# iden3/circom-witnesscalc

Measured on AMD Instinct MI355X. Metric: witnesses/sec, higher is better.
Workload: dtype u32

## Files before the change

### circom-witnesscalc_amd/__init__.py

```python
import ctypes
import os
import subprocess

import numpy as np

_HERE = os.path.dirname(os.path.abspath(__file__))
LIB_PATH = os.environ.get("CWC_LIB_PATH") or os.path.join(_HERE, "libcircom_witnesscalc_amd.so")
_lib = None


class GwStatus(ctypes.Structure):
    _fields_ = [("code", ctypes.c_int), ("error_msg", ctypes.c_void_p)]


class GraphInfo(ctypes.Structure):
    _fields_ = [(n, ctypes.c_uint64) for n in ("n_nodes", "n_op", "n_input_nodes", "n_const", "n_inputs",
                                                "n_witness", "depth", "algorithmic_bytes_per_set")]


class Timing(ctypes.Structure):
    _fields_ = [("tile_width", ctypes.c_uint32), ("n_launches", ctypes.c_uint32), ("n_bundles", ctypes.c_uint64),
                ("n_slots", ctypes.c_uint64), ("interp_ms", ctypes.c_float), ("pack_ms", ctypes.c_float),
                ("divider", ctypes.c_uint32), ("streams", ctypes.c_uint32)]

# ... 17 lines not shown
class Handoff(ctypes.Structure):
    _fields_ = [("struct_size", ctypes.c_uint32), ("form", ctypes.c_uint32), ("hip_stream", ctypes.c_void_p), ("done_event", ctypes.c_void_p)]


FORM_CANONICAL, FORM_MONTGOMERY = 0, 1


class WitnessCalcError(RuntimeError):
    pass


def pinned_rows(shape):
    import weakref
    n = int(np.prod(shape))
    ptr = lib().gwb_host_alloc(n)
    if not ptr:
        raise WitnessCalcError("gwb_host_alloc(%d) failed" % n)
    buf = (ctypes.c_uint8 * max(n, 1)).from_address(ptr)
    weakref.finalize(buf, lib().gwb_host_free, ptr)
    return np.frombuffer(buf, dtype=np.uint8, count=n).reshape(shape)


EXPORTED_SYMBOLS = [
    "gw_calc_witness", "gwb_graph_load", "gwb_graph_free", "gwb_graph_info", "gwb_graph_serialize",
    "gwb_inputs_from_json", "gwb_set_tile_width", "gwb_calc_witness_batch_device", "gwb_calc_witness_batch_host",
    "gwb_last_timing", "gwb_wtns_size", "gwb_wtns_from_witness", "gwb_graph_export", "gwb_graph_import",
    "gwb_free_status", "gwb_profile_classes", "gwb_pick_tile_width", "gwb_inputs_from_json_batch", "gwb_wtns_save_batch",
    "gwb_host_alloc", "gwb_host_free", "gwb_timing_history", "gwb_calc_witness_batch_handoff", "gwb_ubench_modmul", "gwb_graph_pick_tile_width", "gwb_graph_broadcast",
    "gwb_builder_new", "gwb_builder_free", "gwb_builder_input", "gwb_builder_constant", "gwb_builder_uno", "gwb_builder_duo", "gwb_builder_tres",
    "gwb_builder_witness", "gwb_builder_input_signal", "gwb_builder_node_count", "gwb_builder_finish",
    "gwb_ubench_modmul_block", "gwb_program_stats", "gwb_calc_witness_json_to_wtns", "gwb_model_class_cycles",
    "gwb_graphgen_bigint_class", "gwb_graphgen_rsa_long_div_class", "gwb_graph_op_histogram",
    "gwb_kernel_source_hash", "gwb_pack_schedule", "gwb_pack_schedule_of_blob", "gwb_rccl_unique_id", "gwb_rccl_comm_init", "gwb_rccl_comm_ranks", "gwb_rccl_comm_destroy",
]


def build(verbose=False, diag=False):
    cmd = ["make", "-C", os.path.join(_HERE, "csrc"), "-j4"] + (["all", "diag"] if diag else [])
    if not verbose:
        cmd.insert(1, "-s")
    subprocess.check_call(cmd)
    subprocess.check_call(["make"] + ([] if verbose else ["-s"]) + ["-C", os.path.join(_HERE, "r1cs"), "-j4"])


DIAG_LIB_PATH = os.path.join(_HERE, "libcircom_witnesscalc_amd_diag.so")


def lib():
    global _lib
    if _lib is None:
        if not os.path.exists(LIB_PATH):
            raise WitnessCalcError("HIP extension %s is missing: run __graft_entry__.build() "
                                   "(there is no CPU fallback)" % LIB_PATH)
        try:
            import torch
        except ImportError:
            pass
        L = ctypes.CDLL(LIB_PATH)
        vp, sz, u32p = ctypes.c_void_p, ctypes.c_size_t, ctypes.POINTER(ctypes.c_uint32)
        stp = ctypes.POINTER(GwStatus)
        L.gw_calc_witness.restype = ctypes.c_int
        L.gw_calc_witness.argtypes = [ctypes.c_char_p, vp, sz, ctypes.POINTER(vp), ctypes.POINTER(sz), stp]
        L.gwb_graph_load.restype = ctypes.c_int
        L.gwb_graph_load.argtypes = [vp, sz, ctypes.POINTER(vp), stp]
        L.gwb_graph_free.argtypes = [vp]
        L.gwb_graph_info.argtypes = [vp, ctypes.POINTER(GraphInfo)]
        L.gwb_graph_serialize.argtypes = [vp, ctypes.POINTER(vp), ctypes.POINTER(sz), stp]
        L.gwb_inputs_from_json.argtypes = [vp, ctypes.c_char_p, vp, stp]
        L.gwb_set_tile_width.argtypes = [vp, ctypes.c_uint32]
        L.gwb_calc_witness_batch_device.argtypes = [vp, vp, sz, vp, vp, vp, stp]
        L.gwb_calc_witness_batch_host.argtypes = [vp, vp, sz, vp, vp, stp]
        L.gwb_last_timing.argtypes = [vp, ctypes.POINTER(Timing)]
        L.gwb_host_alloc.restype = ctypes.c_void_p
        L.gwb_host_alloc.argtypes = [sz]
        L.gwb_host_free.restype = None
        L.gwb_host_free.argtypes = [ctypes.c_void_p]
        L.gwb_timing_history.restype = ctypes.c_int
        L.gwb_timing_history.argtypes = [ctypes.c_void_p, sz, ctypes.c_void_p, ctypes.c_void_p, ctypes.POINTER(sz)]
        L.gwb_wtns_size.restype = sz
        L.gwb_wtns_size.argtypes = [sz]
        L.gwb_wtns_from_witness.argtypes = [vp, sz, vp]
        L.gwb_graph_export.argtypes = [vp, ctypes.c_uint32, ctypes.POINTER(vp), ctypes.POINTER(sz), stp]
        L.gwb_graph_import.argtypes = [vp, sz, ctypes.POINTER(vp), stp]
        L.gwb_free_status.argtypes = [stp]
        if hasattr(L, "gwb_graphgen_bigint_class"):
            L.gwb_graphgen_bigint_class.argtypes = [ctypes.c_uint32, ctypes.c_uint32, ctypes.c_uint32, ctypes.POINTER(vp), ctypes.POINTER(sz), stp]
            L.gwb_graphgen_rsa_long_div_class.argtypes = [ctypes.c_uint32, ctypes.c_uint32, ctypes.c_uint32, ctypes.c_int, ctypes.POINTER(vp), ctypes.POINTER(sz), stp]
            L.gwb_graph_op_histogram.argtypes = [vp, ctypes.POINTER(ctypes.c_uint64), sz]
        L.gwb_profile_classes.argtypes = [vp, vp, sz, vp, vp, vp, stp]
        L.gwb_inputs_from_json_batch.argtypes = [vp, ctypes.c_char_p, sz, vp, sz, ctypes.POINTER(sz), stp]
        L.gwb_wtns_save_batch.argtypes = [vp, sz, sz, ctypes.c_char_p, stp]
        L.gwb_calc_witness_batch_handoff.argtypes = [vp, vp, sz, vp, vp, ctypes.POINTER(Handoff), stp]
        L.gwb_ubench_modmul.restype = ctypes.c_double
        L.gwb_ubench_modmul.argtypes = [ctypes.c_uint32, ctypes.c_uint32]
        L.gwb_ubench_modmul_block.restype = ctypes.c_double
        L.gwb_model_class_cycles.restype = ctypes.c_double
        L.gwb_kernel_source_hash.restype = ctypes.c_char_p
        L.gwb_kernel_source_hash.argtypes = []
        L.gwb_model_class_cycles.argtypes = [ctypes.c_uint32]
        L.gwb_ubench_modmul_block.argtypes = [ctypes.c_uint32, ctypes.c_uint32]
        L.gwb_program_stats.argtypes = [vp, ctypes.c_uint32, ctypes.POINTER(ProgramStats)]
        if hasattr(L, "gwb_pack_schedule"):
            L.gwb_pack_schedule.argtypes = [vp, ctypes.c_uint32, vp, sz, vp, sz, u32p, u32p, u32p, stp]
            L.gwb_pack_schedule_of_blob.argtypes = [vp, sz, vp, sz, vp, sz, u32p, u32p, u32p, stp]
        L.gwb_calc_witness_json_to_wtns.argtypes = [vp, ctypes.c_char_p, sz, ctypes.c_char_p, sz, ctypes.POINTER(sz), vp, sz, ctypes.POINTER(E2eStats), stp]
        L.gwb_graph_pick_tile_width.restype = ctypes.c_uint32
        L.gwb_graph_pick_tile_width.argtypes = [vp, sz]
        L.gwb_pick_tile_width.restype = ctypes.c_uint32
        L.gwb_pick_tile_width.argtypes = [sz]
        u32 = ctypes.c_uint32
        L.gwb_builder_new.restype = vp
        L.gwb_builder_new.argtypes = []
        L.gwb_builder_free.restype = None
        L.gwb_builder_free.argtypes = [vp]
        for name, args in (("input", [u32]), ("constant", [ctypes.c_char_p, sz]), ("uno", [u32, u32]), ("duo", [u32, u32, u32]), ("tres", [u32, u32, u32, u32])):
            f = getattr(L, "gwb_builder_" + name)
            f.restype = u32
            f.argtypes = [vp] + args
        L.gwb_builder_witness.argtypes = [vp, u32]
        L.gwb_builder_input_signal.argtypes = [vp, ctypes.c_char_p, u32, u32]
        L.gwb_builder_node_count.restype = ctypes.c_uint64
        L.gwb_builder_node_count.argtypes = [vp]
# ... 222 lines not shown
                        done_event.cuda_event if done_event is not None else None)
            rc = lib().gwb_calc_witness_batch_handoff(self._h, d_inputs.data_ptr(), b, d_witness.data_ptr(), d_status.data_ptr(),
                                                      ctypes.byref(h), ctypes.byref(st))
        else:
            rc = lib().gwb_calc_witness_batch_device(self._h, d_inputs.data_ptr(), b, d_witness.data_ptr(),
                                                     d_status.data_ptr(), s.cuda_stream, ctypes.byref(st))
        _check(rc, st)

    def timing_history(self, max_launches):
        a = np.zeros(max_launches, dtype=np.float32)
        b = np.zeros(max_launches, dtype=np.float32)
        n = ctypes.c_size_t(0)
        if lib().gwb_timing_history(self._h, max_launches, a.ctypes.data, b.ctypes.data, ctypes.byref(n)) != 0:
            raise WitnessCalcError("gwb_timing_history failed")
        return a[:n.value], b[:n.value]

    def profile_classes(self, d_inputs, d_witness, d_status):
        out = np.zeros(96, dtype=np.uint64)
        st = GwStatus()
        rc = lib().gwb_profile_classes(self._h, d_inputs.data_ptr(), d_inputs.shape[0], d_witness.data_ptr(),
                                       d_status.data_ptr(), out.ctypes.data, ctypes.byref(st))
        _check(rc, st)
        names = ["INPUT", "MUL", "LIN", "DIV", "CMPZ", "CMPS", "BIT", "IDIVMOD", "TERN", "DIVREQ", "DIVGET", "MULQ"]
        res = {n: tuple(int(x) for x in out[4 * i:4 * i + 4]) for i, n in enumerate(names)}
        res["MULF"] = tuple(int(x) for x in out[64:68])
        res["SCAN"] = tuple(int(x) for x in out[68:72])
        res["_scan_kinds"] = {k: tuple(int(x) for x in out[72 + 4 * i:76 + 4 * i]) for i, k in enumerate(("carry", "division", "convolution", "borrow", "comparison"))}
        res["_sections"] = {"MUL": tuple(int(x) for x in out[48:54]), "LIN": tuple(int(x) for x in out[56:62])}
        res["_issue_part"] = {"MUL": int(out[92]), "LIN": int(out[93])}
        res["_pack"] = {"cycles": int(out[94]), "passes": int(out[95])}
        n = int(out[63])
        res["_waves"] = {"n": n, "max_cycles": int(out[54]), "min_cycles": (1 << 40) - int(out[55]) if n else 0,
                         "mean_cycles": int(out[62]) // n if n else 0}
        return res

    def program_stats(self, key=0):
        ps = ProgramStats()
        if lib().gwb_program_stats(self._h, key, ctypes.byref(ps)) != 0:
            raise WitnessCalcError("gwb_program_stats: no such program")
        n = ps.n_classes
        return {"tile_width": ps.tile_width, "divider": ps.divider, "streams": ps.streams, "n_bundles": ps.n_bundles,
                "n_fused_nodes": ps.n_fused_nodes, "n_scan_steps": ps.n_scan_steps, "n_conv_products": ps.n_conv_products, "chain_floor_cycles": ps.chain_floor_cycles, "model_wave_cycles": ps.model_wave_cycles, "lanes_active_mean": ps.lanes_active_mean, "values_per_bundle_mean": ps.values_per_bundle_mean,
                "class_bundles": {CLASS_NAMES[c]: int(ps.class_bundles[c]) for c in range(n) if ps.class_bundles[c]},
                "class_nodes": {CLASS_NAMES[c]: int(ps.class_nodes[c]) for c in range(n) if ps.class_nodes[c]}}

    def pack_schedule(self, key):
        return _pack_schedule(lambda *a: lib().gwb_pack_schedule(self._h, key, *a))

    def last_timing(self):
        t = Timing()
        if lib().gwb_last_timing(self._h, ctypes.byref(t)) != 0:
            raise WitnessCalcError("gwb_last_timing failed")
        return {n: getattr(t, n) for n, _ in Timing._fields_}


def _pack_schedule(call):
    nw, nr, ni, st = ctypes.c_uint32(), ctypes.c_uint32(), ctypes.c_uint32(), GwStatus()
    _check(call(None, 0, None, 0, ctypes.byref(nw), ctypes.byref(nr), ctypes.byref(ni), ctypes.byref(st)), st)
    order, ready = np.zeros(nw.value, dtype=np.uint32), np.zeros(nr.value, dtype=np.uint32)
    _check(call(order.ctypes.data, order.size, ready.ctypes.data, ready.size, ctypes.byref(nw), ctypes.byref(nr), ctypes.byref(ni), ctypes.byref(st)), st)
    return order, ready, int(ni.value)


def pack_schedule_of_blob(blob):
    blob = bytes(blob)
    return _pack_schedule(lambda *a: lib().gwb_pack_schedule_of_blob(blob, len(blob), *a))
# ... 513 lines not shown
```

### circom-witnesscalc_amd/csrc/capi_batch.cc

```cpp
#include "runtime_internal.hpp"

namespace cwcrt {

int load_graph(const void* data, size_t len, gwb_graph** out, std::string& err) {
    std::unique_ptr<gwb_graph> g(new gwb_graph());
    if (!deserialize_witnesscalc_graph((const uint8_t*)data, len, g->graph, err)) return 1;
    g->has_graph = true;
    Program probe;
    if (!probe_graph(g->graph, probe, err)) return 1;
    g->stats = probe.stats;
    g->n_inputs = probe.n_inputs;
    g->n_witness = probe.n_witness;
    g->inputs = g->graph.inputs;
    g->input_index = g->graph.input_index;
    *out = g.release();
    return 0;
}

}

extern "C" {

void gwb_free_status(gw_status_t* status) {
    if (status && status->error_msg) {
// ... 640 lines not shown
            const double cyc = model_class_cycles((int)c) * (double)p->stats.class_bundles[c];
            const double lanes = (double)p->stats.class_nodes[c] * p->T * ((c == C_MULQ || c == C_MULF) ? (double)COOP_LANES : 1.0);
            wsum += cyc;
            lsum += p->stats.class_bundles[c] ? cyc * lanes / (double)p->stats.class_bundles[c] : 0.0;
            vsum += p->stats.class_bundles[c] ? cyc * (double)p->stats.class_nodes[c] * p->T / (double)p->stats.class_bundles[c] : 0.0;
        }
        out->model_wave_cycles = program_wave_cycles(*p);
        out->lanes_active_mean = wsum > 0 ? lsum / wsum : 0.0;
        out->values_per_bundle_mean = wsum > 0 ? vsum / wsum : 0.0;
        out->n_fused_nodes = p->stats.n_fused_nodes;
        out->chain_floor_cycles = (double)p->stats.chain_floor_cycles;
        out->n_scan_steps = p->stats.n_scan_steps;
        out->n_conv_products = p->stats.n_conv_products;
        return 0;
    } catch (...) {
        return 1;
    }
}

int gwb_timing_history(gwb_graph_t* g, size_t max_launches, float* interp_ms, float* pack_ms, size_t* n_out) {
    if (!g || !n_out || (max_launches && (!interp_ms || !pack_ms))) return 1;
    std::lock_guard<std::mutex> lk(g->mu);
    const size_t n = g->pending.size() < max_launches ? g->pending.size() : max_launches;
    for (size_t i = 0; i < n; ++i) {
        auto& c = g->pending[g->pending.size() - n + i];
        if (hipEventSynchronize(c.after_pack) != hipSuccess || hipEventElapsedTime(&interp_ms[i], c.start, c.after_interp) != hipSuccess ||
            hipEventElapsedTime(&pack_ms[i], c.after_interp, c.after_pack) != hipSuccess)
            return 1;
    }
    *n_out = n;
    return 0;
}

int gwb_profile_classes(gwb_graph_t* g, const void* d_inputs, size_t batch, void* d_witness, uint32_t* d_set_status,
                        uint64_t* out36, gw_status_t* status) {
    return guarded(status, [&]() -> int {
    if (!g || !out36) return fail(status, "null argument");
    if (!gwb_kernels_have_diagnostics())
        return fail(status, "class profiling needs the diagnostic library (make -C circom-witnesscalc_amd/csrc diag; load it with CWC_LIB_PATH=<path of "
                            "libcircom_witnesscalc_amd_diag.so>): the product library carries no stamped interpreter instances");
    std::lock_guard<std::mutex> lk(g->mu);
    std::string err = check_device();
    if (!err.empty()) return fail(status, err);
    unsigned long long* d = nullptr;
    if (hipMalloc(&d, 96 * 8) != hipSuccess || hipMemset(d, 0, 96 * 8) != hipSuccess) return fail(status, "hipMalloc failed");
    g->d_prof = d;
    err = run_device(g, d_inputs, batch, d_witness, d_set_status, nullptr);
    g->d_prof = nullptr;
    if (err.empty() && hipDeviceSynchronize() != hipSuccess) err = "hipDeviceSynchronize failed";
    if (err.empty() && hipMemcpy(out36, d, 96 * 8, hipMemcpyDeviceToHost) != hipSuccess) err = "hipMemcpy failed";
    (void)hipFree(d);
    if (!err.empty()) return fail(status, err);
    set_status(status, OK, "");
    return 0;
    });
}

size_t gwb_wtns_size(size_t n_witness) { return wtns_size(n_witness); }

int gwb_wtns_from_witness(const void* row, size_t n_witness, void* out) {
    if ((!row && n_witness) || !out) return 1;
    wtns_from_witness((const uint8_t*)row, n_witness, (uint8_t*)out);
    return 0;
}

}
```

### circom-witnesscalc_amd/csrc/kernels.hip

```cpp
#include <hip/hip_runtime.h>
#include <stdlib.h>

#include "fr_gfx950.hpp"
#include "scan_gfx950.hpp"
#include "program_dev.h"

namespace cwc {

__device__ __forceinline__ Fr fr_from_u4(const uint4& lo, const uint4& hi) {
    return Fr{{lo.x, lo.y, lo.z, lo.w, hi.x, hi.y, hi.z, hi.w}};
}

__device__ __forceinline__ bool wave_any(bool p) { return __ballot(p) != 0ull; }

struct InterpDims {
    uint32_t n_bundles, n_slots, n_inputs, batch, n_const, n_div_requests, trash_off;
    const uint32_t* div_lanes;
    uint32_t n_streams, stream_first[MAX_STREAMS], stream_count[MAX_STREAMS], stream_div_requests[MAX_STREAMS], stream_cref_first[MAX_STREAMS];
    uint4* pack_out;
    const uint2* pack_entries;
    const uint32_t* pack_ready;
    uint32_t n_inline, pack_mont, n_witness;
};
static const uint32_t ST_DIVIDER_TIMEOUT = 0x80000000u;
// ... 22 lines not shown
    asm volatile("s_mov_b32 m0, %0\n\ts_nop 0\n\tbuffer_load_dwordx4 %1, %2, %3 offen lds"
                 :: "s"(lds_addr), "v"(voff), "s"(rsrc), "s"(soff) : "memory");
}
__device__ __forceinline__ i32x4 make_rsrc_words(const void* base, uint32_t bytes) {
    const uint64_t a = (uint64_t)base;
    return i32x4{(int)(uint32_t)a, (int)((uint32_t)(a >> 32) & 0xffffu), (int)bytes, 0x00020000};
}

template <int T, bool PROF, int W, int PACK, int MODE = 0>
__global__ __launch_bounds__((W > 0 ? (W + 1) * PACK : PACK) * 64) void interp_kernel(const uint32_t* __restrict__ hdr, const uint4* __restrict__ recs,
                                                    const uint32_t* __restrict__ crefs, InterpDims p, WsTable wst,
                                                    const uint4* __restrict__ inputs, uint32_t* __restrict__ status,
                                                    unsigned long long* __restrict__ prof) {
    constexpr int G = 64 / T;
    constexpr bool M2 = MODE == 2 || MODE == 3, WIDE = MODE == 3;
    constexpr uint32_t HI = 16u * T;
    constexpr bool DIVIDER = W > 0;
    constexpr uint32_t NW = (W > 0 ? (uint32_t)W : 1u) * (uint32_t)PACK;
    constexpr uint32_t WD = W > 0 ? (uint32_t)W : 1u;
    constexpr uint32_t AREA = lds_area_bytes((uint32_t)W, LDS_BYTES);
    constexpr uint32_t ML = mbox_lanes((uint32_t)W), MB = mbox_bytes((uint32_t)W);
    const uint32_t batch = p.batch;
    const uint32_t lane = threadIdx.x & 63u;
    const uint32_t wave = (uint32_t)__builtin_amdgcn_readfirstlane((int)(threadIdx.x >> 6));
    const uint32_t n_tiles = (batch + T - 1) / T;
    const uint32_t t = lane % T;
    const uint32_t j = (G == 1) ? 0u : lane / T;
    const uint32_t NS = p.n_streams;
    const uint32_t stream = wave < NW ? wave % NS : 0u;
    const uint32_t tile_raw = blockIdx.x * (NW / NS) + (wave < NW ? wave : 0u) / NS;
    const uint32_t tile = tile_raw < n_tiles ? tile_raw : n_tiles - 1;
    const uint32_t set = tile * T + t;
    const uint32_t set_c = set < batch ? set : batch - 1;
    const uint64_t tile_bytes = ws_tile_bytes(p.n_const, p.n_slots, T);
    const uint32_t chunk = tile / wst.tiles_per_chunk, tile_in_chunk = tile % wst.tiles_per_chunk;
    char* tile_base = reinterpret_cast<char*>(wst.base[chunk]) + (uint64_t)tile_in_chunk * tile_bytes;
    const __amdgpu_buffer_rsrc_t rsrc = __builtin_amdgcn_make_buffer_rsrc(tile_base, 0, (int)(uint32_t)tile_bytes, 0x00020000);
    const i32x4 rsrc_rec = make_rsrc_words(recs, (p.n_bundles + REC_AHEAD) * (uint32_t)G * 16u);
    uint32_t* const sync_words = reinterpret_cast<uint32_t*>(tile_base + ws_sync_offset(p.n_const, p.n_slots, T));
    static_assert(NW + PACK <= 16, "sequence words: 64 bytes");
    __shared__ uint4 lds[(NW * AREA + (DIVIDER ? NW * MB + 64u : 0u)) / 16];
    const uint32_t area = wave * AREA;
    const uint32_t lds0 = (uint32_t)(uintptr_t)(lds_char*)(char*)lds + area;
    const uint32_t t16 = 16u * t, lane16 = 16u * lane, j16 = 16u * j;
    char* const ldsb = reinterpret_cast<char*>(lds) + area;
    char* const mbox_all = reinterpret_cast<char*>(lds) + NW * AREA;
    char* const mbox = mbox_all + (wave < NW ? wave : 0u) * MB;
    volatile uint32_t* const seq = reinterpret_cast<volatile uint32_t*>(mbox_all + NW * MB);
    if (DIVIDER || NW > 1) {
        if (DIVIDER && threadIdx.x < NW + (uint32_t)PACK) seq[threadIdx.x] = 0;
        if (NS > 1 && wave < NW && stream == 0 && lane < MAX_STREAMS && tile_raw < n_tiles) {
            __hip_atomic_store(sync_words + lane, 0u, __ATOMIC_RELAXED, __HIP_MEMORY_SCOPE_AGENT);
            __builtin_amdgcn_fence(__ATOMIC_RELEASE, "agent");
        }
        if (wave < NW && stream == 0 && j == 0 && tile_raw < n_tiles && set < batch) status[set] = 0;
        __syncthreads();
    } else {
        if (j == 0 && tile_raw < n_tiles && set < batch) status[set] = 0;
    }
    if (DIVIDER) {
        if (wave >= NW) {
            const uint32_t first_w = (wave - NW) * WD, first_tile = blockIdx.x * (NW / NS) + first_w / NS;
            if (first_tile >= n_tiles) return;
            const uint32_t n_active = NS > 1 ? 1u : n_tiles - first_tile < WD ? n_tiles - first_tile : WD;
            char* const mbox_d = mbox_all + first_w * MB;
            const uint32_t n_requests = NS > 1 ? p.stream_div_requests[first_w % NS] : p.n_div_requests;
// ... 70 lines not shown
                    break;
                }
                __builtin_amdgcn_fence(__ATOMIC_ACQUIRE, "workgroup");
                const uint32_t lanes_k = p.div_lanes[div_lanes_base + k];
                const uint32_t total = n_active * lanes_k;
                for (uint32_t g0 = 0; g0 < total; g0 += 64u) {
                    const uint32_t g = g0 + lane;
                    const bool valid = g < total;
                    const uint32_t w = valid ? g / lanes_k : 0u, i = valid ? g % lanes_k : 0u;
                    char* mb = mbox_d + w * MB + 16u * i;
                    const uint4* qa = reinterpret_cast<const uint4*>(mb);
                    const uint4* qb = reinterpret_cast<const uint4*>(mb + 32u * ML);
                    Fr a = fr_from_u4(qa[0], qa[ML]), b = fr_from_u4(qb[0], qb[ML]);
                    if (!valid) b = fr_zero();
                    const Fr inv = fr_inv(b);
                    const Fr r = u256_select(u256_is_zero(b), fr_zero(), fr_mul(a, inv));
                    if (valid) {
                        uint4* qr = reinterpret_cast<uint4*>(mb);
                        qr[0] = make_uint4(r.v[0], r.v[1], r.v[2], r.v[3]);
                        qr[ML] = make_uint4(r.v[4], r.v[5], r.v[6], r.v[7]);
                    }
                }
                __builtin_amdgcn_fence(__ATOMIC_RELEASE, "workgroup");
                if (lane == 0) seq[wave] = k + 1;
            }
            if constexpr (W == 1) {
                if (inl) {
                    pk_run(p.pack_ready[n_requests] < p.n_inline ? p.pack_ready[n_requests] : p.n_inline, 0xffffffffu);
                    if (PROF && lane == 0 && first_tile % 64u == 0) {
                        atomicAdd(&prof[94], pk_cycles);
                        atomicAdd(&prof[95], pk_passes);
                    }
                }
            }
            return;
        }
    }
    if (tile_raw >= n_tiles) return;
    uint32_t div_seq = 0;
    uint32_t n_posts = 0, n_waits = 0;
    uint32_t cref_row = p.stream_cref_first[stream];

    auto ld = [&](uint32_t off) -> Fr {
        const u32x4 lo = __builtin_amdgcn_raw_buffer_load_b128(rsrc, (int)off, 0, 0);
        const u32x4 hi = __builtin_amdgcn_raw_buffer_load_b128(rsrc, (int)off + (int)HI, 0, 0);
        return Fr{{lo.x, lo.y, lo.z, lo.w, hi.x, hi.y, hi.z, hi.w}};
    };
    auto ld_lds = [&](uint32_t addr) -> Fr {
        const uint4* q = reinterpret_cast<const uint4*>(ldsb + addr);
        const uint4 lo = q[0], hi = q[LDS_HALF_BYTES / 16];
        return fr_from_u4(lo, hi);
    };
    auto ld_rec2 = [&](uint32_t bundle, uint32_t half) -> uint2 {
        return *reinterpret_cast<const uint2*>(ldsb + LDS_REC_OFF + (bundle % REC_AHEAD) * REC_BYTES + lane16 + 8u * half);
    };
    const uint32_t B0 = p.stream_first[stream], NBND = B0 + p.stream_count[stream];
    if (NBND == B0) return;
    auto clampb = [&](uint32_t b) { return b < NBND ? b : NBND - 1; };
    auto stage_rec = [&](uint32_t bundle) {
        dma16(lds0 + LDS_REC_OFF + (bundle % REC_AHEAD) * REC_BYTES, j16, rsrc_rec, bundle * (uint32_t)G * 16u);
    };
    constexpr uint32_t DMA_BIAS = 3u * LDS_HALF_BYTES;
    const i32x4 rsrc_dma = make_rsrc_words(tile_base - DMA_BIAS, (uint32_t)tile_bytes + DMA_BIAS);
    const uint32_t dma_soff0 = DMA_BIAS, dma_soff1 = DMA_BIAS + HI - LDS_HALF_BYTES, dma_soff2 = DMA_BIAS - 2u * LDS_HALF_BYTES,
                   dma_soff3 = DMA_BIAS + HI - 3u * LDS_HALF_BYTES;
    static_assert(LDS_HALF_BYTES == 1024, "instruction offsets below are written out");
// ... 766 lines not shown
                const uint32_t cr = crefs[(size_t)cref_row * G + j];
                ++cref_row;
                const Fr y = ld(cr + t16);
                r = u256_select(u256_is_zero(a_op), y, b_op);
                break;
            }
            case C_SYNC: {
                r = fr_zero();
                if (h & HDR_POST) {
                    asm volatile("s_waitcnt vmcnt(0)" ::: "memory");
                    ++n_posts;
                    if (lane == 0) __hip_atomic_store(sync_words + stream, n_posts, __ATOMIC_RELEASE, __HIP_MEMORY_SCOPE_AGENT);
                }
                if (h & HDR_WAIT) {
                    ++n_waits;
                    if (!post_wait(sync_words, n_waits)) err_bits |= ST_SYNC_TIMEOUT;
                }
                break;
            }
            case C_SCAN: r = fr_zero(); break;
            default: r = fr_zero(); break;
        }
        finish(r);
    }
    __builtin_amdgcn_raw_buffer_store_b128(u32x4{r_prev.v[0], r_prev.v[1], r_prev.v[2], r_prev.v[3]}, rsrc, (int)doff_prev, 0, 0);
    __builtin_amdgcn_raw_buffer_store_b128(u32x4{r_prev.v[4], r_prev.v[5], r_prev.v[6], r_prev.v[7]}, rsrc, (int)doff_prev + (int)HI, 0, 0);
    if (PROF && lane == 0) {
        const unsigned long long cyc = __builtin_amdgcn_s_memtime() - t_wave0;
        atomicMax(&prof[54], cyc);
        atomicMax(&prof[55], (1ull << 40) - cyc);
        atomicAdd(&prof[62], cyc);
        atomicAdd(&prof[63], 1ull);
    }
    if (PROF && lane == 0 && (tile % 64u) == 0u) {
#pragma unroll
        for (int c = 0; c < C_PROF; ++c) {
            atomicAdd(&prof[c * 4 + 0], pf[c][0]);
            atomicAdd(&prof[c * 4 + 3], pf[c][1]);
        }
        atomicAdd(&prof[M2 ? 68 : 64], pf_fused[0]);
        atomicAdd(&prof[M2 ? 71 : 67], pf_fused[1]);
        if (M2) {
#pragma unroll
            for (int q = 0; q < 5; ++q) {
                atomicAdd(&prof[72 + 4 * q], pf_scan[q][0]);
                atomicAdd(&prof[75 + 4 * q], pf_scan[q][1]);
            }
        }
#pragma unroll
        for (int k = 0; k < 2; ++k)
#pragma unroll
            for (int q = 0; q < 6; ++q) atomicAdd(&prof[48 + 8 * k + q], psec[k][q]);
        atomicAdd(&prof[92], psec[0][6]);
        atomicAdd(&prof[93], psec[1][6]);
    }
    if (err_bits && set < batch) atomicOr(&status[set], err_bits);
}

__global__ __launch_bounds__(256) void fill_consts_kernel(ProgramDev p, WsTable wst, uint32_t n_tiles, uint32_t T) {
    const uint32_t e = blockIdx.x * 256u + threadIdx.x;
    const uint32_t pieces = p.n_const * 2u * T;
    if (e >= pieces) return;
    const uint4 v = reinterpret_cast<const uint4*>(p.consts)[(size_t)(e / (2u * T)) * 2u + (e / T) % 2u];
    const uint64_t tile_bytes = ws_tile_bytes(p.n_const, p.n_slots, T);
    for (uint32_t tile = blockIdx.y; tile < n_tiles; tile += gridDim.y) {
        char* tb = reinterpret_cast<char*>(wst.base[tile / wst.tiles_per_chunk]) + (uint64_t)(tile % wst.tiles_per_chunk) * tile_bytes;
// ... 270 lines not shown
```

### circom-witnesscalc_amd/csrc/pipeline.cc

```cpp
#include "runtime_internal.hpp"

namespace cwcrt {


void set_status(gw_status_t* st, GW_ERROR_CODE code, const std::string& msg) {
    if (!st) return;
    st->code = code;
    if (code == OK && msg.empty()) {
        st->error_msg = nullptr;
        return;
    }
    st->error_msg = (char*)malloc(msg.size() + 1);
    if (st->error_msg) memcpy(st->error_msg, msg.c_str(), msg.size() + 1);
}
int fail(gw_status_t* st, const std::string& msg) {
    set_status(st, ERROR, msg);
    return 1;
}
std::string upload_program(DeviceProgram& dp) {
    const Program& p = dp.host;
    auto al = [](size_t x) { return (x + 255) & ~(size_t)255; };
    const size_t o_hdr = 0, o_recs = o_hdr + al(p.hdr.size() * 4 + 16), o_crefs = o_recs + al(p.recs.size() * 4 + REC_AHEAD * 1024u),
                 o_consts = o_crefs + al(p.crefs.size() * 4 + 256), o_wit = o_consts + al(p.consts.size() * 4 + 32),
                 o_div = o_wit + al(p.witness_refs.size() * 4 + 4), o_order = o_div + al(p.div_lanes.size() * 4 + 4),
// ... 30 lines not shown
    if (dp.dev.has_fused == 2u)
        for (uint32_t h : p.hdr)
            if ((h & HDR_CLASS_MASK) == C_SCAN && !(h & HDR_SCAN_CONV) &&
                ((h & (HDR_SCAN_BORROW | HDR_SCAN_LEX)) || (!(h & HDR_SCAN_DIV) && ((h >> HDR_SCAN_SHIFT_SHIFT) & 0xffu) != 64u))) {
                dp.dev.has_fused = 3u;
                break;
            }
    {
        const PackSchedule& sc = dp.sched;
        std::vector<uint32_t> entries(sc.order.size() * 2);
        for (size_t i = 0; i < sc.order.size(); ++i) {
            entries[2 * i] = sc.order[i];
            entries[2 * i + 1] = p.witness_refs[sc.order[i]];
        }
        if (!sc.order.empty()) HIP_TRY(hipMemcpy(d + o_order, sc.order.data(), sc.order.size() * 4, hipMemcpyHostToDevice));
        if (!entries.empty()) HIP_TRY(hipMemcpy(d + o_entries, entries.data(), entries.size() * 4, hipMemcpyHostToDevice));
        HIP_TRY(hipMemcpy(d + o_ready, sc.ready.data(), sc.ready.size() * 4, hipMemcpyHostToDevice));
        dp.dev.pack_order = (const uint32_t*)(d + o_order);
        dp.dev.pack_entries = (const uint32_t*)(d + o_entries);
        dp.dev.pack_ready = (const uint32_t*)(d + o_ready);
        dp.dev.n_inline = sc.n_inline;
        dp.dev.n_ready_last = sc.ready.back();
    }
    dp.dev.n_streams = p.n_streams;
    for (uint32_t s = 0; s < MAX_STREAMS; ++s) {
        dp.dev.stream_first[s] = p.stream_first[s];
        dp.dev.stream_count[s] = p.stream_count[s];
        dp.dev.stream_div_requests[s] = p.stream_div_requests[s];
        dp.dev.stream_cref_first[s] = p.stream_cref_first[s];
    }
    return "";
}

uint32_t waves_per_workgroup(uint32_t divider, uint64_t tiles, uint32_t streams) {
    if (streams > 1) return divider ? streams : 4u;
    const char* e = getenv("CWC_WAVES_PER_WORKGROUP");
    if (divider == 1) return e ? (atoi(e) >= 4 ? 2u : 1u) : (tiles > 256 ? 2u : 1u);
    if (divider) return 1;
    if (e) return atoi(e) == 4 ? 4u : 1u;
    return tiles > 512 ? 4u : 1u;
}

uint64_t workspace_budget() {
    const char* e = getenv("CWC_WORKSPACE_GB");
    double gb = e ? atof(e) : 8.0;
    if (gb < 1e-4) gb = 1e-4;
    return (uint64_t)(gb * (double)(1ull << 30));
}
}

extern "C" uint32_t gwb_pick_tile_width(size_t batch) {
    size_t target = 2048, divider_tiles = 1024;
    if (const char* e = getenv("CWC_TARGET_WAVES")) {
        long v = atol(e);
        if (v > 0) target = (size_t)v;
    }
    if (const char* e = getenv("CWC_DIVIDER_TILES")) divider_tiles = (size_t)atol(e);
    uint32_t t = batch <= 256 ? 1 : batch <= 1024 ? 2 : 4;
    while (t < 64 && (batch + t - 1) / t > target) t *= 2;
    const size_t tiles = (batch + t - 1) / t;
    return t | (tiles <= divider_tiles && t < 64 ? KEY_DIVIDER : 0u);
}

namespace cwcrt {

std::string check_device() {
    int n = 0;
    hipError_t e = hipGetDeviceCount(&n);
    if (e != hipSuccess || n <= 0)
        return std::string("no HIP device available (") + (e != hipSuccess ? hipGetErrorString(e) : "device count 0") +
               "); this library has no CPU fallback";
    static const std::string xnack_refusal = []() -> std::string {
        int dev = 0;
        hipDeviceProp_t prop;
        if (hipGetDevice(&dev) != hipSuccess || hipGetDeviceProperties(&prop, dev) != hipSuccess) {
            (void)hipGetLastError();
            return "";
        }
        return strstr(prop.gcnArchName, "xnack+") ? std::string("device ") + prop.gcnArchName + ": XNACK-enabled devices are not supported (run with HSA_XNACK=0)" : "";
    }();
    return xnack_refusal;
}

double estimate_cycles(const Program& p, size_t batch) {
    const double wide = p.T >= 8 ? 1.10 : 1.0;
    if (p.n_streams > 1) {
        const double tiles = (double)((batch + p.T - 1) / p.T);
        const double t = program_wave_cycles(p);
        double busy = 0;
        for (uint32_t s = 0; s < p.n_streams; ++s) busy += (p.stream_cycles[s] + model_class_cycles(C_DIV) * p.stream_div_requests[s]) / t;
        const double wgs = p.divider ? tiles : std::ceil(tiles * p.n_streams / 4.0);
        const double wg_per_cu = p.divider ? (p.n_streams == 4 ? 1.0 : 3.0) : 2.0;
        const double rounds = std::max(1.0, wgs / (256.0 * wg_per_cu));
        const double crowd = std::max(1.0, 1.1 * (tiles / rounds) * busy / 1024.0);
        return t * (p.T >= 4 ? 1.2 * wide : p.T == 2 ? 1.08 : 1.0) * crowd * rounds;
    }
    const double per_wave = program_wave_cycles(p) * wide;
    const double heavy = program_wave_cycles_mul_div(p) * wide;
    const double waves = (double)((batch + p.T - 1) / p.T);
    const double two_per_simd = (1.3 * heavy + 1.9 * (per_wave - heavy)) / per_wave;
    if (p.divider == 4) return per_wave * 1.30 * (waves <= 1024 ? 1.0 : waves / 1024);
    if (p.divider == 3) return per_wave * 1.08 * (waves <= 768 ? 1.0 : two_per_simd * (waves <= 1536 ? 1.0 : waves / 1536));
    const double resident = waves * (p.divider == 1 ? 2.0 : 1.0);
    double crowd = resident <= 1024 ? 1.0 : two_per_simd;
    if (p.divider == 1 && resident > 1024) crowd = 1.0 + 0.75 * (crowd - 1.0);
    const double rounds = resident <= 2048 ? 1.0 : resident / 2048;
    return per_wave * crowd * rounds;
}

std::vector<uint32_t> candidate_keys(const ProgramStats& stats, size_t batch, uint32_t rule, uint32_t min_t) {
    size_t divider_tiles = 1024;
    if (const char* e = getenv("CWC_DIVIDER_TILES")) divider_tiles = (size_t)atol(e);
    const bool has_div = stats.class_nodes[C_DIV] > 0;
    const uint32_t t0 = rule & ~KEY_MODE_MASK;
    std::vector<uint32_t> keys;
    for (uint32_t t = std::max(min_t, t0 >= 4 ? t0 / 4 : 1u); t <= t0 * 2 && t <= 32 && (batch >= 64 || t == t0); t *= 2)
        for (uint32_t mode : {0u, KEY_DIVIDER, KEY_TRIPLE, KEY_GROUP}) {
            const size_t tiles = (batch + t - 1) / t;
            if (tiles > 4 * 2048) continue;
            const bool divider_fits = has_div && tiles <= divider_tiles;
            if (mode == 0 && divider_fits) continue;
            if (mode == KEY_DIVIDER && !divider_fits) continue;
            if (mode == KEY_TRIPLE && !(has_div && tiles > 512 && tiles <= 768 && !getenv("CWC_NO_GROUP_DIVIDER"))) continue;
            if (mode == KEY_GROUP && !(has_div && tiles > 512 && tiles <= 1024 && !getenv("CWC_NO_GROUP_DIVIDER"))) continue;
            keys.push_back(t | mode);
            if ((mode == 0 || mode == KEY_DIVIDER) && t < 64 && !getenv("CWC_NO_STREAMS")) {
                if (tiles <= 256) keys.push_back(t | mode | KEY_STREAMS4);
                else if (tiles <= 340) keys.push_back(t | mode | KEY_STREAMS2);
            }
        }
    return keys;
}

gwb_graph::Refined refine_choice(const Graph& graph, const ProgramStats& stats, size_t batch, uint32_t rule, uint32_t min_t) {
    gwb_graph::Refined r;
    try {
        double best_cost = -1;
        std::unique_ptr<SharedRewrites, void (*)(SharedRewrites*)> rewrites(make_shared_rewrites(), free_shared_rewrites);
        for (uint32_t key : candidate_keys(stats, batch, rule, min_t)) {
            std::unique_ptr<Program> p(new Program());
            std::string err;
            if (!compile_program(graph, key & ~KEY_MODE_MASK, key_divider_waves(key), *p, err, key_streams(key), false, rewrites.get())) continue;
            const double cost = estimate_cycles(*p, batch);
            if (best_cost < 0 || cost < best_cost) {
                best_cost = cost;
                r.best = key;
            }
            r.programs[key] = std::move(p);
        }
    } catch (...) {
        r.best = 0;
        r.programs.clear();
    }
    return r;
}

uint32_t pick_tile_width(gwb_graph* g, size_t batch, bool allow_quick) {
    if (!g->has_graph && !g->progs.empty()) return g->progs.begin()->first;
    if (g->forced_T) return g->forced_T;
    if (const char* e = getenv("CWC_TILE_WIDTH")) {
        const uint32_t key = (uint32_t)atoi(e), t = key & ~KEY_MODE_MASK;
// ... 448 lines not shown
```

### circom-witnesscalc_amd/csrc/program_dev.h

```cpp
#pragma once
#include <stdint.h>

#include "ops.h"

#if defined(__HIPCC__)
#define CWC_HD __host__ __device__ static inline
#define CWC_HDC __host__ __device__ static constexpr
#else
#define CWC_HD static inline
#define CWC_HDC static constexpr
#endif

namespace cwc {

enum BundleClass : uint32_t {
    C_INPUT = 0,
    C_MUL = 1,
    C_LIN = 2,
    C_DIV = 3,
    C_CMPZ = 4,
    C_CMPS = 5,
    C_BIT = 6,
    C_IDIVMOD = 7,
    C_TERN = 8,
    C_DIVREQ = 9,
    C_DIVGET = 10,
    C_MULQ = 11,
    C_SYNC = 12,
    C_MULF = 13,
    C_SCAN = 14,
    C_COUNT = 15
};
static const uint32_t COOP_LANES = 4, COOP_MAX_T = 4, COOP_FUSE_MAX_T = 2, SCAN_MAX_T = 2;
static const uint32_t HDR_SCAN_DIV = 1u << 11, HDR_SCAN_CONV = 1u << 12;
enum SelCode : uint32_t { SEL_LT = 1, SEL_GT = 2, SEL_LEQ = 3, SEL_GEQ = 4, SEL_NEZ = 5, SEL_OUT_MONT = 8 };
static const uint32_t HDR_SCAN_BORROW = 1u << 13, HDR_SCAN_LEX = 1u << 14, HDR_SCAN_KG = 1u << 15, HDR_SCAN_KL = 1u << 16;
static const int HDR_SCAN_SHIFT_SHIFT = 19, HDR_SCAN_ITER_SHIFT = 27;
static const uint32_t SCAN_ROLE_ACC = 1u, SCAN_START = 2u;
enum FusedOp : uint32_t { FOP_NONE = 0, FOP_MUL = 1, FOP_ADD = 2, FOP_SUB = 3 , FOP_RSUB = 4  };
static const uint32_t HDR_F_S2MUL = 1u << 11, HDR_F_S2LIN = 1u << 12, HDR_F_S3LIN = 1u << 13;
CWC_HDC uint32_t coop_nodes(uint32_t T) { return T <= COOP_MAX_T ? 64u / (COOP_LANES * T) : 0u; }

static const uint32_t OFF_NOWHERE = 0xffff0000u;
static const uint32_t HDR_CLASS_MASK = 0xfu;
static const int HDR_COUNT_SHIFT = 4;
static const uint32_t HDR_LIN_SUB = 1u << 11, HDR_LIN_ADD = 1u << 12, HDR_BITX_ALL = 1u << 13;
static const uint32_t HDR_MUL_CC = 1u << 13;
static const uint32_t HDR_BIT_ALL_SHR = 1u << 11, HDR_BIT_ALL_BAND = 1u << 12;
static const uint32_t HDR_B_CANON = 1u << 14, HDR_A_CANON = 1u << 17, HDR_OUT_CANON = 1u << 18;
static const uint32_t HDR_POST = 1u << 15, HDR_WAIT = 1u << 16;
static const uint32_t MAX_STREAMS = 4;
static const uint32_t CTRL_SUB_MASK = 7u, CTRL_ACTIVE = 8u, CTRL_MASK = 15u;
static const uint32_t RING_BUNDLES = 4, OPND_AHEAD = 2, REC_AHEAD = 4;
static const uint32_t RING_SLOT_BYTES = 2048, LDS_HALF_BYTES = 1024, STAGE_BYTES = 4096, REC_BYTES = 1024;
CWC_HDC uint32_t mbox_lanes(uint32_t W) { return W <= 1u ? 64u : 32u; }
CWC_HDC uint32_t mbox_bytes(uint32_t W) { return mbox_lanes(W) * 64u; }
CWC_HDC uint32_t lds_area_bytes(uint32_t W, uint32_t lds_bytes) { return (void)W, lds_bytes; }
static const uint32_t LDS_RING_OFF = 0, LDS_STAGE_OFF = LDS_RING_OFF + RING_BUNDLES * RING_SLOT_BYTES,
                      LDS_REC_OFF = LDS_STAGE_OFF + OPND_AHEAD * STAGE_BYTES, LDS_BYTES = LDS_REC_OFF + REC_AHEAD * REC_BYTES;
enum SubOp : uint32_t {
    SUB_ADD = 0, SUB_SUB = 1, SUB_MULT = 2,
    SUB_EQ = 0, SUB_NEQ = 1, SUB_LAND = 2, SUB_LOR = 3,
    SUB_LT = 0, SUB_GT = 1, SUB_LEQ = 2, SUB_GEQ = 3,
    SUB_SHL = 0, SUB_SHR = 1, SUB_BOR = 2, SUB_BAND = 3, SUB_BXOR = 4,
    SUB_BITX = 5,
    SUB_IDIV = 0, SUB_MOD = 1,
};

static const uint32_t REF_CONST = 0x80000000u;
static const uint32_t REF_CANON = 0x40000000u;

enum SetStatus : uint32_t {
    ST_SHL_OVERFLOW = 1u,
    ST_BITOP_EQ_R = 2u,
};

struct ProgramDev {
    const uint32_t* hdr;
    const uint32_t* recs;
    const uint32_t* crefs;
    const uint32_t* consts;
    const uint32_t* witness_refs;
    const uint32_t* div_lanes;
    uint32_t n_bundles, n_slots, n_inputs, n_witness, n_const;
// ... 22 lines not shown
```

### include/graph_witness_batch.h

```cpp
#ifndef CWC_AMD_GRAPH_WITNESS_BATCH_H
#define CWC_AMD_GRAPH_WITNESS_BATCH_H

#include <stddef.h>
#include <stdint.h>

#include "graph_witness.h"

#ifdef __cplusplus
extern "C" {
#endif

typedef struct gwb_graph gwb_graph_t;

typedef struct {
  uint64_t n_nodes;
  uint64_t n_op;
  uint64_t n_input_nodes;
  uint64_t n_const;
  uint64_t n_inputs;
  uint64_t n_witness;
  uint64_t depth;
  uint64_t algorithmic_bytes_per_set;
} gwb_graph_info_t;

// ... 50 lines not shown
                                  size_t *n_sets, uint32_t *set_status, size_t max_sets, gwb_e2e_stats_t *stats, gw_status_t *status);

#define GWB_TILE_ASYNC_DIVIDER 0x100u
#define GWB_TILE_GROUP_DIVIDER 0x200u
#define GWB_TILE_TRIPLE_DIVIDER 0x400u
#define GWB_TILE_STREAMS2 0x800u
#define GWB_TILE_STREAMS4 0x1000u
int gwb_set_tile_width(gwb_graph_t *g, uint32_t tile_width);
uint32_t gwb_pick_tile_width(size_t batch);
uint32_t gwb_graph_pick_tile_width(gwb_graph_t *g, size_t batch);

int gwb_calc_witness_batch_device(gwb_graph_t *g, const void *d_inputs, size_t batch, void *d_witness,
                                  uint32_t *d_set_status, void *hip_stream, gw_status_t *status);
#define GWB_FORM_CANONICAL 0u
#define GWB_FORM_MONTGOMERY 1u
typedef struct {
  uint32_t struct_size;
  uint32_t form;
  void *hip_stream;
  void *done_event;
} gwb_handoff_t;
int gwb_calc_witness_batch_handoff(gwb_graph_t *g, const void *d_inputs, size_t batch, void *d_witness,
                                   uint32_t *d_set_status, const gwb_handoff_t *handoff, gw_status_t *status);

int gwb_calc_witness_batch_host(gwb_graph_t *g, const void *inputs, size_t batch, void *witness,
                                uint32_t *set_status, gw_status_t *status);
void *gwb_host_alloc(size_t bytes);
void gwb_host_free(void *p);
int gwb_last_timing(gwb_graph_t *g, gwb_timing_t *t);
int gwb_timing_history(gwb_graph_t *g, size_t max_launches, float *interp_ms, float *pack_ms, size_t *n_out);

int gwb_profile_classes(gwb_graph_t *g, const void *d_inputs, size_t batch, void *d_witness,
                        uint32_t *d_set_status, uint64_t *out64, gw_status_t *status);

double gwb_ubench_modmul(uint32_t waves_per_simd, uint32_t iters);

double gwb_ubench_modmul_block(uint32_t waves_per_simd, uint32_t iters);
double gwb_model_class_cycles(uint32_t bundle_class);
const char* gwb_kernel_source_hash(void);

typedef struct {
  uint32_t tile_width, divider, streams, n_classes;
  uint64_t n_bundles, n_fused_nodes;
  uint64_t class_bundles[16];
  uint64_t class_nodes[16];
  double model_wave_cycles;
  double lanes_active_mean;
  double values_per_bundle_mean;
  double chain_floor_cycles;
  uint64_t n_scan_steps;
  uint64_t n_conv_products;
} gwb_program_stats_t;
int gwb_program_stats(gwb_graph_t *g, uint32_t program_key, gwb_program_stats_t *out);

int gwb_pack_schedule(gwb_graph_t *g, uint32_t program_key, uint32_t *pack_order, size_t order_cap, uint32_t *pack_ready, size_t ready_cap,
                      uint32_t *n_witness, uint32_t *n_ready, uint32_t *n_inline, gw_status_t *status);
int gwb_pack_schedule_of_blob(const void *blob, size_t blob_len, uint32_t *pack_order, size_t order_cap, uint32_t *pack_ready, size_t ready_cap,
                              uint32_t *n_witness, uint32_t *n_ready, uint32_t *n_inline, gw_status_t *status);

size_t gwb_wtns_size(size_t n_witness);
int gwb_wtns_from_witness(const void *witness_row, size_t n_witness, void *out);

int gwb_graph_export(gwb_graph_t *g, uint32_t tile_width, void **blob, size_t *blob_len, gw_status_t *status);
int gwb_graph_import(const void *blob, size_t blob_len, gwb_graph_t **out, gw_status_t *status);

#define GWB_RCCL_UNIQUE_ID_BYTES 128
// ... 14 lines not shown
```

Before: 88360.

## Pair two stream tiles per workgroup for divider dual-stream programs and add wave census

Adds a new dual-stream candidate key for divider programs with 340-512 tiles and, when streams=2 with a divider, launches four waves per workgroup so two tiles share a workgroup. A matching cost model is added so the autotuner can pick this configuration against the existing keys. Separately adds a diagnostic-only wave census (hardware IDs and timestamps per wave) for profiling builds. The intent is better SIMD occupancy and overlap for mid-size batches; the risk is the model misranking the new key.

```diff
diff --git a/circom-witnesscalc_amd/__init__.py b/circom-witnesscalc_amd/__init__.py
--- a/circom-witnesscalc_amd/__init__.py
+++ b/circom-witnesscalc_amd/__init__.py
@@ -73,6 +73,7 @@
     "gwb_ubench_modmul_block", "gwb_program_stats", "gwb_calc_witness_json_to_wtns", "gwb_model_class_cycles",
     "gwb_graphgen_bigint_class", "gwb_graphgen_rsa_long_div_class", "gwb_graph_op_histogram",
     "gwb_kernel_source_hash", "gwb_pack_schedule", "gwb_pack_schedule_of_blob", "gwb_rccl_unique_id", "gwb_rccl_comm_init", "gwb_rccl_comm_ranks", "gwb_rccl_comm_destroy",
+    "gwb_wave_census",
 ]
 
 
@@ -129,6 +130,8 @@
             L.gwb_graphgen_rsa_long_div_class.argtypes = [ctypes.c_uint32, ctypes.c_uint32, ctypes.c_uint32, ctypes.c_int, ctypes.POINTER(vp), ctypes.POINTER(sz), stp]
             L.gwb_graph_op_histogram.argtypes = [vp, ctypes.POINTER(ctypes.c_uint64), sz]
         L.gwb_profile_classes.argtypes = [vp, vp, sz, vp, vp, vp, stp]
+        if hasattr(L, "gwb_wave_census"):
+            L.gwb_wave_census.argtypes = [vp, vp, sz, vp, vp, vp, sz, stp]
         L.gwb_inputs_from_json_batch.argtypes = [vp, ctypes.c_char_p, sz, vp, sz, ctypes.POINTER(sz), stp]
         L.gwb_wtns_save_batch.argtypes = [vp, sz, sz, ctypes.c_char_p, stp]
         L.gwb_calc_witness_batch_handoff.argtypes = [vp, vp, sz, vp, vp, ctypes.POINTER(Handoff), stp]
@@ -417,6 +420,22 @@
         n = int(out[63])
         res["_waves"] = {"n": n, "max_cycles": int(out[54]), "min_cycles": (1 << 40) - int(out[55]) if n else 0,
                          "mean_cycles": int(out[62]) // n if n else 0}
+        return res
+
+    def wave_census(self, d_inputs, d_witness, d_status):
+        out = np.zeros(3 * 8192, dtype=np.uint64)
+        st = GwStatus()
+        rc = lib().gwb_wave_census(self._h, d_inputs.data_ptr(), d_inputs.shape[0], d_witness.data_ptr(),
+                                   d_status.data_ptr(), out.ctypes.data, out.size, ctypes.byref(st))
+        _check(rc, st)
+        rec = out.reshape(-1, 3)
+        idx = [i for i in range(rec.shape[0]) if rec[i, 1]]
+        res = []
+        for i in idx:
+            w0 = int(rec[i, 0])
+            role, wpw = (w0 >> 40) & 255, (w0 >> 48) & 255
+            res.append({"workgroup": i // wpw, "wave": i % wpw, "xcc": (w0 >> 32) & 15, "se": (w0 >> 13) & 7, "sh": (w0 >> 12) & 1, "cu": (w0 >> 8) & 15, "simd": (w0 >> 4) & 3,
+                        "divider": role & 1, "stream": (role >> 1) & 7, "has_tile": (role >> 4) & 1, "start": int(rec[i, 1]), "end": int(rec[i, 2])})
         return res
 
     def program_stats(self, key=0):
diff --git a/circom-witnesscalc_amd/csrc/capi_batch.cc b/circom-witnesscalc_amd/csrc/capi_batch.cc
--- a/circom-witnesscalc_amd/csrc/capi_batch.cc
+++ b/circom-witnesscalc_amd/csrc/capi_batch.cc
@@ -696,27 +696,47 @@
     return 0;
 }
 
-int gwb_profile_classes(gwb_graph_t* g, const void* d_inputs, size_t batch, void* d_witness, uint32_t* d_set_status,
-                        uint64_t* out36, gw_status_t* status) {
-    return guarded(status, [&]() -> int {
-    if (!g || !out36) return fail(status, "null argument");
+static int run_stamped(gwb_graph_t* g, const void* d_inputs, size_t batch, void* d_witness, uint32_t* d_set_status, uint64_t* counters,
+                       uint64_t* census, gw_status_t* status) {
     if (!gwb_kernels_have_diagnostics())
         return fail(status, "class profiling needs the diagnostic library (make -C circom-witnesscalc_amd/csrc diag; load it with CWC_LIB_PATH=<path of "
                             "libcircom_witnesscalc_amd_diag.so>): the product library carries no stamped interpreter instances");
     std::lock_guard<std::mutex> lk(g->mu);
     std::string err = check_device();
     if (!err.empty()) return fail(status, err);
+    const size_t census_bytes = (size_t)CENSUS_MAX_WAVES * CENSUS_WORDS * 8, bytes = PROF_WORDS * 8 + census_bytes;
     unsigned long long* d = nullptr;
-    if (hipMalloc(&d, 96 * 8) != hipSuccess || hipMemset(d, 0, 96 * 8) != hipSuccess) return fail(status, "hipMalloc failed");
+    if (hipMalloc(&d, bytes) != hipSuccess) return fail(status, "hipMalloc failed");
+    if (hipMemset(d, 0, bytes) != hipSuccess) {
+        (void)hipFree(d);
+        return fail(status, "hipMemset failed");
+    }
     g->d_prof = d;
     err = run_device(g, d_inputs, batch, d_witness, d_set_status, nullptr);
     g->d_prof = nullptr;
     if (err.empty() && hipDeviceSynchronize() != hipSuccess) err = "hipDeviceSynchronize failed";
-    if (err.empty() && hipMemcpy(out36, d, 96 * 8, hipMemcpyDeviceToHost) != hipSuccess) err = "hipMemcpy failed";
+    if (err.empty() && counters && hipMemcpy(counters, d, PROF_WORDS * 8, hipMemcpyDeviceToHost) != hipSuccess) err = "hipMemcpy failed";
+    if (err.empty() && census && hipMemcpy(census, d + PROF_WORDS, census_bytes, hipMemcpyDeviceToHost) != hipSuccess) err = "hipMemcpy failed";
     (void)hipFree(d);
     if (!err.empty()) return fail(status, err);
     set_status(status, OK, "");
     return 0;
+}
+
+int gwb_profile_classes(gwb_graph_t* g, const void* d_inputs, size_t batch, void* d_witness, uint32_t* d_set_status,
+                        uint64_t* out36, gw_status_t* status) {
+    return guarded(status, [&]() -> int {
+    if (!g || !out36) return fail(status, "null argument");
+    return run_stamped(g, d_inputs, batch, d_witness, d_set_status, out36, nullptr, status);
+    });
+}
+
+int gwb_wave_census(gwb_graph_t* g, const void* d_inputs, size_t batch, void* d_witness, uint32_t* d_set_status,
+                    uint64_t* out, size_t out_words, gw_status_t* status) {
+    return guarded(status, [&]() -> int {
+    if (!g || !out) return fail(status, "null argument");
+    if (out_words < (size_t)CENSUS_MAX_WAVES * CENSUS_WORDS) return fail(status, "gwb_wave_census: the output buffer is too small");
+    return run_stamped(g, d_inputs, batch, d_witness, d_set_status, nullptr, out, status);
     });
 }
 
diff --git a/circom-witnesscalc_amd/csrc/kernels.hip b/circom-witnesscalc_amd/csrc/kernels.hip
--- a/circom-witnesscalc_amd/csrc/kernels.hip
+++ b/circom-witnesscalc_amd/csrc/kernels.hip
@@ -78,6 +78,20 @@
     const uint32_t tile = tile_raw < n_tiles ? tile_raw : n_tiles - 1;
     const uint32_t set = tile * T + t;
     const uint32_t set_c = set < batch ? set : batch - 1;
+    [[maybe_unused]] auto census_slot = [&]() -> unsigned long long* {
+        const uint32_t wv = blockIdx.x * (blockDim.x >> 6) + wave;
+        return lane == 0 && wv < CENSUS_MAX_WAVES ? prof + PROF_WORDS + CENSUS_WORDS * wv : nullptr;
+    };
+    if constexpr (PROF) {
+        if (unsigned long long* c = census_slot()) {
+            const uint32_t w_of = wave < NW ? wave : (wave - NW) * WD;
+            const uint32_t has_tile = blockIdx.x * (NW / NS) + w_of / NS < n_tiles ? 1u : 0u;
+            const unsigned long long role = (wave >= NW ? 1u : 0u) | (w_of % NS) << 1 | has_tile << 4 | (blockDim.x >> 6) << 8;
+            constexpr int HWREG_HW_ID = 4 | 31 << 11, HWREG_XCC_ID = 20 | 31 << 11;
+            c[0] = (unsigned long long)__builtin_amdgcn_s_getreg(HWREG_HW_ID) | (unsigned long long)(__builtin_amdgcn_s_getreg(HWREG_XCC_ID) & 15u) << 32 | role << 40;
+            c[1] = __builtin_amdgcn_s_memtime();
+        }
+    }
     const uint64_t tile_bytes = ws_tile_bytes(p.n_const, p.n_slots, T);
     const uint32_t chunk = tile / wst.tiles_per_chunk, tile_in_chunk = tile % wst.tiles_per_chunk;
     char* tile_base = reinterpret_cast<char*>(wst.base[chunk]) + (uint64_t)tile_in_chunk * tile_bytes;
@@ -214,6 +228,9 @@
                         atomicAdd(&prof[95], pk_passes);
                     }
                 }
+            }
+            if constexpr (PROF) {
+                if (unsigned long long* c = census_slot()) c[2] = __builtin_amdgcn_s_memtime();
             }
             return;
         }
@@ -1046,6 +1063,9 @@
         atomicAdd(&prof[62], cyc);
         atomicAdd(&prof[63], 1ull);
     }
+    if constexpr (PROF) {
+        if (unsigned long long* c = census_slot()) c[2] = __builtin_amdgcn_s_memtime();
+    }
     if (PROF && lane == 0 && (tile % 64u) == 0u) {
 #pragma unroll
         for (int c = 0; c < C_PROF; ++c) {
diff --git a/circom-witnesscalc_amd/csrc/pipeline.cc b/circom-witnesscalc_amd/csrc/pipeline.cc
--- a/circom-witnesscalc_amd/csrc/pipeline.cc
+++ b/circom-witnesscalc_amd/csrc/pipeline.cc
@@ -86,7 +86,13 @@
     return "";
 }
 
+static bool stream_pair_workgroups(uint32_t divider, uint64_t tiles, uint32_t streams) {
+    if (streams != 2 || divider != 1) return false;
+    if (const char* e = getenv("CWC_STREAM_TILES_PER_WORKGROUP")) return atoi(e) == 2;
+    return tiles > 256;
+}
 uint32_t waves_per_workgroup(uint32_t divider, uint64_t tiles, uint32_t streams) {
+    if (stream_pair_workgroups(divider, tiles, streams)) return 4u;
     if (streams > 1) return divider ? streams : 4u;
     const char* e = getenv("CWC_WAVES_PER_WORKGROUP");
     if (divider == 1) return e ? (atoi(e) >= 4 ? 2u : 1u) : (tiles > 256 ? 2u : 1u);
@@ -140,6 +146,17 @@
     const double wide = p.T >= 8 ? 1.10 : 1.0;
     if (p.n_streams > 1) {
         const double tiles = (double)((batch + p.T - 1) / p.T);
+        if (stream_pair_workgroups(p.divider, (uint64_t)tiles, p.n_streams)) {
+            constexpr double kTwoWaves = 0.62, kPackCyclesPerValue = 0.028;
+            double t = 0;
+            for (uint32_t s = 0; s < p.n_streams; ++s) {
+                const double own = std::max(p.stream_cycles[s], p.stream_chain_cycles[s]);
+                const double simd = (p.stream_cycles[s] + model_class_cycles(C_DIV) * p.stream_div_requests[s]) * kTwoWaves;
+                t = std::max(t, std::max(own, simd));
+            }
+            const double rounds = std::max(1.0, tiles / 512.0);
+            return t * (p.T >= 4 ? 1.2 * wide : 1.0) * rounds + kPackCyclesPerValue * (double)p.n_witness * (double)batch;
+        }
         const double t = program_wave_cycles(p);
         double busy = 0;
         for (uint32_t s = 0; s < p.n_streams; ++s) busy += (p.stream_cycles[s] + model_class_cycles(C_DIV) * p.stream_div_requests[s]) / t;
@@ -181,6 +198,8 @@
             if ((mode == 0 || mode == KEY_DIVIDER) && t < 64 && !getenv("CWC_NO_STREAMS")) {
                 if (tiles <= 256) keys.push_back(t | mode | KEY_STREAMS4);
                 else if (tiles <= 340) keys.push_back(t | mode | KEY_STREAMS2);
+                else if (mode == KEY_DIVIDER && t >= 2 && tiles <= 512 && !getenv("CWC_INLINE_PACK") && !getenv("CWC_INLINE_PACK_ROWS"))
+                    keys.push_back(t | mode | KEY_STREAMS2);
             }
         }
     return keys;
diff --git a/circom-witnesscalc_amd/csrc/program_dev.h b/circom-witnesscalc_amd/csrc/program_dev.h
--- a/circom-witnesscalc_amd/csrc/program_dev.h
+++ b/circom-witnesscalc_amd/csrc/program_dev.h
@@ -50,6 +50,7 @@
 static const uint32_t HDR_B_CANON = 1u << 14, HDR_A_CANON = 1u << 17, HDR_OUT_CANON = 1u << 18;
 static const uint32_t HDR_POST = 1u << 15, HDR_WAIT = 1u << 16;
 static const uint32_t MAX_STREAMS = 4;
+static const uint32_t PROF_WORDS = 96, CENSUS_MAX_WAVES = 8192, CENSUS_WORDS = 3;
 static const uint32_t CTRL_SUB_MASK = 7u, CTRL_ACTIVE = 8u, CTRL_MASK = 15u;
 static const uint32_t RING_BUNDLES = 4, OPND_AHEAD = 2, REC_AHEAD = 4;
 static const uint32_t RING_SLOT_BYTES = 2048, LDS_HALF_BYTES = 1024, STAGE_BYTES = 4096, REC_BYTES = 1024;
diff --git a/include/graph_witness_batch.h b/include/graph_witness_batch.h
--- a/include/graph_witness_batch.h
+++ b/include/graph_witness_batch.h
@@ -106,6 +106,8 @@
 
 int gwb_profile_classes(gwb_graph_t *g, const void *d_inputs, size_t batch, void *d_witness,
                         uint32_t *d_set_status, uint64_t *out64, gw_status_t *status);
+int gwb_wave_census(gwb_graph_t *g, const void *d_inputs, size_t batch, void *d_witness,
+                    uint32_t *d_set_status, uint64_t *out64, size_t out_words, gw_status_t *status);
 
 double gwb_ubench_modmul(uint32_t waves_per_simd, uint32_t iters);
 
```

After: 93500, median of 6. 1.06x the previous value.
